# zhaoweicai/mscnn

Measured on AMD Instinct MI355X. Metric: images/sec mscnn-7s-576 KITTI-car inference, higher is better.
Workload: dtype f32

## Files before the change

### include/mscnn_hip.h

```cpp
#ifndef MSCNN_HIP_H_
#define MSCNN_HIP_H_

#include <stddef.h>
#include <stdint.h>

#if defined(__GNUC__)
#define MSCNN_API __attribute__((visibility("default")))
#else
#define MSCNN_API
#endif

#ifdef __cplusplus
extern "C" {
#endif

typedef enum {
  MSCNN_OK = 0,
  MSCNN_ERR_BAD_ARG = 1,
  MSCNN_ERR_HIP = 2,
  MSCNN_ERR_WORKSPACE = 3,
  MSCNN_ERR_UNSUPPORTED = 4
} mscnn_status;

MSCNN_API const char* mscnn_last_error(void);
// ... 31 lines not shown
MSCNN_API int mscnn_conv2d_plan_plane_columns(const mscnn_conv_plan* plan, int* cols, int n);
MSCNN_API int mscnn_conv2d_plan_set_profiling(mscnn_conv_plan* plan, int on);
MSCNN_API int mscnn_conv2d_plan_stage_ms(const mscnn_conv_plan* plan, float ms_out[3]);
#define MSCNN_AMAX_SLOTS 1024
MSCNN_API int mscnn_conv2d_plan_publishes_amax(const mscnn_conv_plan* plan);
MSCNN_API int mscnn_conv2d_plan_set_amax_io(mscnn_conv_plan* plan, const uint32_t* in_bound, uint32_t* out_amax);
MSCNN_API int mscnn_conv2d_plan_set_batch(mscnn_conv_plan* plan, int N);
MSCNN_API unsigned long long mscnn_conv2d_plan_weight_layout(const mscnn_conv_plan* plan);
MSCNN_API int mscnn_conv2d_pack_weights(const mscnn_conv_plan* plan, const float* w, float* packed, void* stream);
MSCNN_API int mscnn_conv2d_fwd_f32(const mscnn_conv_plan* plan, const float* x, const float* w, const float* packed,
                         const float* bias, float* y, void* workspace, size_t workspace_bytes, void* stream);
MSCNN_API int mscnn_conv2d_plan_can_pool(const mscnn_conv_plan* plan);
MSCNN_API int mscnn_conv2d_fwd_pool_f32(const mscnn_conv_plan* plan, const float* x, const float* w, const float* packed,
                              const float* bias, float* y, float* y_pool, void* workspace, size_t workspace_bytes,
                              void* stream);

MSCNN_API int mscnn_relu_fwd_f32(const float* x, float* y, size_t count, float negative_slope, void* stream);

MSCNN_API int mscnn_pool_out_dim(int in, int kernel, int pad, int stride);
MSCNN_API int mscnn_pool2d_fwd_f32(const float* x, float* y, int N, int C, int H, int W, int kernel_h, int kernel_w,
                         int pad_h, int pad_w, int stride_h, int stride_w, int method, void* stream);

MSCNN_API int mscnn_inner_product_fwd_f32(const float* x, const float* w, const float* bias, float* y,
                                int M, int N, int K, int relu, void* stream);
MSCNN_API void mscnn_debug_inner_product_rows(int rows);

MSCNN_API int mscnn_inner_product_wg_supported(int M, int N, int K);
MSCNN_API size_t mscnn_inner_product_wg_packed_bytes(int N, int K);
MSCNN_API size_t mscnn_inner_product_wg_workspace_bytes(int M, int N, int K);
MSCNN_API int mscnn_inner_product_wg_pack(const float* w, float* wt, int N, int K, void* stream);
MSCNN_API int mscnn_inner_product_wg_fwd(const float* x, const float* wt, const float* bias, float* y, int M, int N, int K, int relu,
                                         void* workspace, size_t workspace_bytes, void* stream);
MSCNN_API unsigned long long mscnn_wgemm_handoff_event(void);
MSCNN_API void mscnn_wgemm_force_whole_tiles(int on);
MSCNN_API int mscnn_wgemm_whole_tiles_forced(void);
MSCNN_API void mscnn_debug_wgemm_handoff_fault(int drop_publish, unsigned spin_limit);
MSCNN_API long mscnn_debug_wgemm_schedule(const mscnn_conv_plan* plan, int whole_tiles, int* rows, long max_rows, int info[8]);
MSCNN_API int mscnn_inner_product_x3_supported(int N, int K);
MSCNN_API size_t mscnn_inner_product_x3_packed_bytes(int N, int K);
MSCNN_API size_t mscnn_inner_product_x3_workspace_bytes(int M, int N, int K);
MSCNN_API int mscnn_inner_product_x3_pack(const float* w, void* packed, int N, int K, void* stream);
MSCNN_API int mscnn_inner_product_x3_fwd(const float* x, const void* packed, const float* bias, float* y, int M, int N, int K, int relu,
                               const uint32_t* in_bound, void* workspace, size_t workspace_bytes, void* stream);
MSCNN_API int mscnn_inner_product_f16_supported(int N, int K);
MSCNN_API int mscnn_inner_product_pack_f16(const float* w, void* w16, int N, int K, void* stream);
MSCNN_API int mscnn_inner_product_fwd_f16(const float* x, const void* w16, const float* bias, float* y, int M, int N, int K, int relu,
                                          void* stream);

MSCNN_API int mscnn_concat_channels_f32(const float* x, float* y, int N, int C, int inner, int C_total, int c_offset, void* stream);

MSCNN_API int mscnn_deconv_depthwise_fwd_f32(const float* x, const float* w, const float* bias, float* y,
                                   int N, int C, int H, int W, int Kh, int Kw, int pad_h, int pad_w,
                                   int stride_h, int stride_w, void* stream);

MSCNN_API int mscnn_deconv2d_fwd_f32(const float* x, const float* w, const float* bias, float* y, int N, int Cin, int H, int W,
                                     int Cout, int Kh, int Kw, int pad_h, int pad_w, int stride_h, int stride_w, int group,
                                     void* stream);

MSCNN_API int mscnn_max_rel_diff_f32(const float* a, const float* ref, size_t count, float floor, float* out_dev, void* stream);
MSCNN_API int mscnn_max_rel_diff_strided_f32(const float* a, size_t a_stride, const float* ref, size_t ref_stride, size_t planes, size_t run,
                                             const double* sumsq_dev, double sumsq_count, float* out_dev, void* stream);
MSCNN_API int mscnn_store_words_i32(int* dst_dev, const int* values_host, int n, void* stream);
MSCNN_API int mscnn_sum_squares_f32(const float* x, size_t count, double* out_dev, void* stream);

MSCNN_API int mscnn_softmax_fwd_f32(const float* x, float* y, int outer, int C, int inner, void* stream);

MSCNN_API int mscnn_roipool_fwd_f32(const float* feat, const float* rois, float* out, int R, int N, int C, int H, int W,
                          int pooled_h, int pooled_w, float spatial_scale, float pad_ratio,
                          int C_total, int c_offset, void* stream);
MSCNN_API int mscnn_roipool_pair_fwd_f32(const float* feat, const float* rois, float* out, int R, int N, int C, int H, int W,
                                         int pooled_h, int pooled_w, float spatial_scale, float pad_ratio_a, int c_offset_a,
                                         float pad_ratio_b, int c_offset_b, int C_total, void* stream);

MSCNN_API int mscnn_conv2d_plan_can_chain(const mscnn_conv_plan* plan, const mscnn_conv_plan* next);
MSCNN_API int mscnn_conv2d_plan_can_pool_only(const mscnn_conv_plan* plan);
MSCNN_API int mscnn_conv2d_fwd_chain_f32(const mscnn_conv_plan* plan, const mscnn_conv_plan* next, const float* x, const float* packed,
                               const float* bias, float* y, float* y_pool, void* workspace, size_t workspace_bytes,
                               void* next_workspace, size_t next_workspace_bytes, void* stream);

MSCNN_API int mscnn_conv2d_plan_can_fuse_roipool(const mscnn_conv_plan* plan, int C, int pooled_h, int pooled_w);
MSCNN_API size_t mscnn_conv2d_roipool_workspace_bytes(const mscnn_conv_plan* plan, int N, int C, int H, int W);
MSCNN_API size_t mscnn_roipool_maps_bytes(int N, int C, int H, int W);
MSCNN_API int mscnn_roipool_maps_build_f32(const float* feat, float* maps, int N, int C, int H, int W, void* stream);
MSCNN_API int mscnn_conv2d_fwd_roipool_pair_f32(const mscnn_conv_plan* plan, const float* feat, const float* prepared_maps, int N, int C,
                                                int H, int W, const float* rois, float spatial_scale, float pad_ratio_a,
                                                float pad_ratio_b, const float* packed_w, const float* bias, float* y, void* workspace,
                                                size_t workspace_bytes, void* stream);

MSCNN_API int mscnn_roialign_fwd_f32(const float* feat, const float* rois, float* out, int R, int N, int C, int H, int W,
                                     int pooled_h, int pooled_w, float spatial_scale, float pad_ratio, void* stream);
MSCNN_API int mscnn_roialign_ave_fwd_f32(const float* feat, const float* rois, float* out, int R, int N, int C, int H, int W,
                                         int pooled_h, int pooled_w, float spatial_scale, float pad_ratio,
                                         int C_total, int c_offset, void* stream);
MSCNN_API int mscnn_roialign_ave_pair_fwd_f32(const float* feat, const float* rois, float* out, int R, int N, int C, int H, int W,
                                              int pooled_h, int pooled_w, float spatial_scale, float pad_ratio_a, int c_offset_a,
                                              float pad_ratio_b, int c_offset_b, int C_total, void* stream);

MSCNN_API int mscnn_eltwise_fwd_f32(const float* const* bottoms_host, int num_bottoms, const float* coeffs_host, float* y,
                                    size_t count, int op, void* stream);

#define MSCNN_BOXOUT_MAX_HEADS 16
typedef struct {
  int num_heads;
  int num;
  int channels;
  int head_h[MSCNN_BOXOUT_MAX_HEADS], head_w[MSCNN_BOXOUT_MAX_HEADS];
  float field_w[MSCNN_BOXOUT_MAX_HEADS], field_h[MSCNN_BOXOUT_MAX_HEADS], downsample_rate[MSCNN_BOXOUT_MAX_HEADS];
  float fg_thr, iou_thr;
  int nms_mode;
  float field_whr, field_xyr;
  int max_nms_num, max_post_nms_num;
  float min_size;
  int do_bbox_norm;
  float bbox_mean[4], bbox_std[4];
} mscnn_boxoutput_desc;

MSCNN_API size_t mscnn_boxoutput_workspace_bytes(const mscnn_boxoutput_desc* desc);
MSCNN_API int mscnn_boxoutput_max_rows(const mscnn_boxoutput_desc* desc);
MSCNN_API int mscnn_boxoutput_fwd_f32(const mscnn_boxoutput_desc* desc, const float* const* heads_host,
                            float* rois_out, float* props_out, int* anchor_ids_out, int cap,
                            int* count_out_dev, void* workspace, size_t workspace_bytes, void* stream);
MSCNN_API size_t mscnn_boxoutput_batch_workspace_bytes(const mscnn_boxoutput_desc* desc);
MSCNN_API int mscnn_boxoutput_batch_fwd_f32(const mscnn_boxoutput_desc* desc, const float* const* heads_host,
                            float* rois_out, float* props_out, int* anchor_ids_out, int cap,
                            int* count_out_dev, void* workspace, size_t workspace_bytes, void* stream);

MSCNN_API size_t mscnn_nms_workspace_bytes(int n);
MSCNN_API int mscnn_nms_greedy_f32(const float* boxes_xywh, int n, float iou_thr, int nms_mode, unsigned char* keep_out,
                         void* workspace, size_t workspace_bytes, void* stream);

MSCNN_API int mscnn_decodebbox_fwd_f32(const float* bbox, const float* prior, float* out, int R, int bbox_dim,
                             const float* mean_host, const float* std_host, void* stream);

typedef struct {
  int ncls, cls_id;
  float bbox_mean[4], bbox_std[4];
  float proposal_thr;
  double ratio_h, ratio_w, org_h, org_w, nms_overlap;
} mscnn_detections_desc;
MSCNN_API size_t mscnn_detections_workspace_bytes(int R);

enum { MSCNN_NMS_TYPE_MAXG = 0, MSCNN_NMS_TYPE_MAX = 1, MSCNN_NMS_TYPE_MS = 2, MSCNN_NMS_TYPE_COVER = 3, MSCNN_NMS_TYPE_NONE = 4 };
enum { MSCNN_NMS_OVR_UNION = 0, MSCNN_NMS_OVR_MIN = 1 };
#ifndef MSCNN_NMS_PARAMS_DEFINED
#define MSCNN_NMS_PARAMS_DEFINED
typedef struct {
  int type;
  int ovr_dnm;
  double thr;
  float det_thr;
} mscnn_nms_params;
#endif
MSCNN_API int mscnn_nms_params_resolve(const mscnn_nms_params* nms, mscnn_nms_params* out);
MSCNN_API int mscnn_nms_params_from_names(const char* type, const char* ovr_dnm, double thr, double maxn, float det_thr,
                                          mscnn_nms_params* out);
MSCNN_API int mscnn_detections_fwd(const mscnn_detections_desc* desc, const float* bbox_pred, const float* cls_pred,
                         const float* props, int R, double* dets_out, int* ids_out, int* count_out_dev,
                         void* workspace, size_t workspace_bytes, void* stream);

MSCNN_API int mscnn_detections_nms_fwd(const mscnn_detections_desc* desc, const mscnn_nms_params* nms, const float* bbox_pred,
                                       const float* cls_pred, const float* props, int R, double* dets_out, int* ids_out,
                                       int* count_out_dev, void* workspace, size_t workspace_bytes, void* stream);

MSCNN_API int mscnn_detections_cascade_fwd(const mscnn_detections_desc* desc, float det_thr, const float* boxes,
                                 const float* cls_prob, const float* props, int R, double* dets_out, int* ids_out,
                                 int* count_out_dev, void* workspace, size_t workspace_bytes, void* stream);
// ... 123 lines not shown
```

### mscnn_amd/csrc/roipool_wino.hip

```cpp
#include "roipool_wino.h"
#include "wino33_device.h"
#include <cfloat>

namespace {

typedef unsigned u32x4 __attribute__((ext_vector_type(4)));
typedef unsigned u32x2 __attribute__((ext_vector_type(2)));

constexpr int kNB = 4;
constexpr int kLevels = 4;

struct RpwArgs {
  const float* maps;
  const float* rois;
  float* V;
  int R, C, H, W, T_pad;
  unsigned level_bytes, maps_bytes, v_bytes;
  float spatial_scale, pad_a, pad_b;
};

__device__ __forceinline__ __amdgpu_buffer_rsrc_t make_rsrc(const void* p, unsigned bytes) {
  return __builtin_amdgcn_make_buffer_rsrc(const_cast<void*>(p), 0, (int)bytes, 0x00020000);
}
__device__ __forceinline__ int uni(int v) { return __builtin_amdgcn_readfirstlane(v); }
// ... 157 lines not shown
      }
      __syncthreads();
#pragma unroll
      for (int j = 0; j < 5; ++j) {
        float* slot_ = &s_out[(j * 64 + lane) * kLdsRow + wave * 4];
        if (!RAG || (i < 4 && j < 4)) *reinterpret_cast<float4*>(slot_) = make_float4(out[j][0], out[j][1], out[j][2], out[j][3]);
        else if (i < 4) *reinterpret_cast<float2*>(slot_) = make_float2(out[j][0], out[j][2]);
        else if (j < 4) *reinterpret_cast<float2*>(slot_) = make_float2(out[j][0], out[j][1]);
        else *slot_ = out[j][0];
      }
      __syncthreads();
      static_assert(kRois == 8, "thread = (channel, roi) of a pass");
#pragma unroll
      for (int j = 0; j < 5; ++j) {
        const int rq = tid % kRois, ch = tid / kRois;
        if (r0 + rq < a.R) {
          const float* unit = &s_out[(j * 64 + ch) * kLdsRow + rq * 4];
          const int uw = RAG ? (i < 4 ? 2 : 1) * (j < 4 ? 2 : 1) : 4;
          const unsigned off = (unsigned)(i * 5 + j) * plane_bytes + ((unsigned)(q * C + c0 + ch) * (unsigned)a.T_pad + (unsigned)(r0 + rq) * (unsigned)uw) * 4u;
#ifdef RPW_NO_STORE
          if (a.T_pad < 0)
#endif
          {
            if (uw == 4) {
              const float4 u = *reinterpret_cast<const float4*>(unit);
              u32x4 pk;
              pk.x = __builtin_bit_cast(unsigned, u.x); pk.y = __builtin_bit_cast(unsigned, u.y);
              pk.z = __builtin_bit_cast(unsigned, u.z); pk.w = __builtin_bit_cast(unsigned, u.w);
              __builtin_amdgcn_raw_buffer_store_b128(pk, rV, off, 0u, 0);
            } else if (uw == 2) {
              const float2 u = *reinterpret_cast<const float2*>(unit);
              u32x2 pk;
              pk.x = __builtin_bit_cast(unsigned, u.x); pk.y = __builtin_bit_cast(unsigned, u.y);
              __builtin_amdgcn_raw_buffer_store_b64(pk, rV, off, 0u, 0);
            } else {
              __builtin_amdgcn_raw_buffer_store_b32(__builtin_bit_cast(unsigned, unit[0]), rV, off, 0u, 0);
            }
          }
        }
      }
    }
  }
}

__global__ __launch_bounds__(256) void nchw_to_nhwc_kernel(const float* __restrict__ x, float* __restrict__ y, int C, int HW) {
  __shared__ float t[64][65];
  const int n = blockIdx.z, c0 = blockIdx.y * 64, p0 = blockIdx.x * 64;
  const int tx = threadIdx.x & 63, ty = threadIdx.x >> 6;
  const float* src = x + (size_t)n * C * HW;
  float* dst = y + (size_t)n * C * HW;
#pragma unroll
  for (int i = 0; i < 16; ++i) {
    const int cc = c0 + ty + 4 * i, pp = p0 + tx;
    t[ty + 4 * i][tx] = (cc < C && pp < HW) ? src[(size_t)cc * HW + pp] : 0.f;
  }
  __syncthreads();
#pragma unroll
  for (int i = 0; i < 16; ++i) {
    const int pp = p0 + ty + 4 * i, cc = c0 + tx;
    if (pp < HW && cc < C) dst[(size_t)pp * C + cc] = t[tx][ty + 4 * i];
  }
}

__global__ __launch_bounds__(256) void sliding_max_kernel(const float* __restrict__ src, float* __restrict__ dst, int H, int W, int C4, int half,
                                                          long total) {
  const long i = blockIdx.x * 256L + threadIdx.x;
  if (i >= total) return;
  const int c4 = (int)(i % C4);
  long p = i / C4;
  const int x = (int)(p % W); p /= W;
  const int y = (int)(p % H);
  const long n = p / H;
  const int y2 = min(y + half, H - 1), x2 = min(x + half, W - 1);
  const float4* s4 = reinterpret_cast<const float4*>(src) + n * H * W * C4;
  const float4 a = s4[((long)y * W + x) * C4 + c4], b = s4[((long)y * W + x2) * C4 + c4];
  const float4 c = s4[((long)y2 * W + x) * C4 + c4], d = s4[((long)y2 * W + x2) * C4 + c4];
  float4 m = a;
  m.x = b.x > m.x ? b.x : m.x; m.y = b.y > m.y ? b.y : m.y; m.z = b.z > m.z ? b.z : m.z; m.w = b.w > m.w ? b.w : m.w;
  m.x = c.x > m.x ? c.x : m.x; m.y = c.y > m.y ? c.y : m.y; m.z = c.z > m.z ? c.z : m.z; m.w = c.w > m.w ? c.w : m.w;
  m.x = d.x > m.x ? d.x : m.x; m.y = d.y > m.y ? d.y : m.y; m.z = d.z > m.z ? d.z : m.z; m.w = d.w > m.w ? d.w : m.w;
  reinterpret_cast<float4*>(dst)[i] = m;
}

}

namespace mscnn {

bool roipool_wino33_supported(int C, int pooled_h, int pooled_w, int conv_pad_h, int conv_pad_w) {
  return pooled_h == 7 && pooled_w == 7 && conv_pad_h == 0 && conv_pad_w == 0 && C > 0 && C % 64 == 0;
}

size_t roipool_wino33_scratch_bytes(int N, int C, int H, int W) { return (size_t)kLevels * N * C * H * W * sizeof(float); }

int roipool_wino33_build_maps(const float* feat, float* maps, int N, int C, int H, int W, hipStream_t st) {
  MSCNN_REQUIRE(feat && maps, "roipool maps: null pointer");
  MSCNN_REQUIRE(N > 0 && C % 64 == 0 && H > 0 && W > 0, "roipool maps: bad shape");
  MSCNN_REQUIRE(kLevels * (double)N * C * H * W * 4.0 < 4.0e9, "roipool maps: beyond a 32-bit buffer window");
  MSCNN_REQUIRE(reinterpret_cast<uintptr_t>(maps) % 16 == 0, "roipool maps: the maps must be 16-byte aligned");
  const int HW = H * W;
  const long per_level = (long)N * C * HW;
  nchw_to_nhwc_kernel<<<dim3(cdiv(HW, 64), cdiv(C, 64), N), 256, 0, st>>>(feat, maps, C, HW);
  MSCNN_POST_LAUNCH();
  for (int k = 1; k < kLevels; ++k) {
    const long total = per_level / 4;
    sliding_max_kernel<<<(unsigned)((total + 255) / 256), 256, 0, st>>>(maps + (k - 1) * per_level, maps + k * per_level, H, W, C / 4, 1 << (k - 1), total);
    MSCNN_POST_LAUNCH();
  }
  return MSCNN_OK;
}

int roipool_wino33_forward(const float* maps, const float* rois, float* V, int R, int N, int C, int H, int W, int T_pad,
                           float spatial_scale, float pad_a, float pad_b, hipStream_t st, int ragged) {
  MSCNN_REQUIRE(maps && rois && V, "roipool+transform: null pointer");
  MSCNN_REQUIRE(ragged == 0 || ragged == wino33_ragged_mode(5, 5), "roipool+transform: the planes are uniform or ragged on both axes (5 x 5 outputs)");
  MSCNN_REQUIRE(R > 0 && N > 0 && C % 64 == 0 && H > 0 && W > 0 && T_pad >= 4 * R && T_pad % 4 == 0, "roipool+transform: bad shape");
  const double lb = (double)N * C * H * W * 4.0, vb = 25.0 * 2.0 * C * (double)T_pad * 4.0;
  MSCNN_REQUIRE(kLevels * lb < 4.0e9 && vb < 4.0e9, "roipool+transform: feature maps or transform planes beyond a 32-bit buffer window");
  MSCNN_REQUIRE(reinterpret_cast<uintptr_t>(V) % 16 == 0, "roipool+transform: V must be 16-byte aligned");
  RpwArgs a;
  a.maps = maps; a.rois = rois; a.V = V;
  a.R = R; a.C = C; a.H = H; a.W = W; a.T_pad = T_pad;
  a.level_bytes = (unsigned)lb; a.maps_bytes = (unsigned)(kLevels * lb); a.v_bytes = (unsigned)vb;
  a.spatial_scale = spatial_scale; a.pad_a = pad_a; a.pad_b = pad_b;
  if (ragged) roipool_wino33_kernel<7, 7, true><<<dim3(C / 64, cdiv(R, kRois), 2), kRois * 64, 0, st>>>(a);
  else roipool_wino33_kernel<7, 7, false><<<dim3(C / 64, cdiv(R, kRois), 2), kRois * 64, 0, st>>>(a);
  MSCNN_POST_LAUNCH();
  return MSCNN_OK;
}

}
```

### mscnn_amd/hipapi.py

```python
import ctypes as C
import os

import numpy as np
import torch

_HERE = os.path.dirname(os.path.abspath(__file__))
LIB_PATH = os.path.join(_HERE, "libmscnn_hip.so")
_lib = None


class MscnnError(RuntimeError):
    pass


class ConvDesc(C.Structure):
    _fields_ = [(n, C.c_int) for n in ("N", "Cin", "H", "W", "Cout", "Kh", "Kw", "pad_h", "pad_w",
                                       "stride_h", "stride_w", "group", "relu", "algo", "tune_variant", "tune_grid", "tune_flags")]


AMAX_SLOTS = 1024
ALGO_AUTO, ALGO_DIRECT, ALGO_WINO_F2, ALGO_WINO_F3, ALGO_F16, ALGO_WINO_F3_X3, ALGO_WINO_F4 = 0, 1, 2, 3, 4, 5, 6


MAX_HEADS = 16
# ... 41 lines not shown
NMS_NULL = object()


def _nms_ref(nms):
    if nms is NMS_NULL:
        return None
    return C.byref(nms if isinstance(nms, NmsParams) else nms_params(**nms))


def lib():
    global _lib
    if _lib is None:
        if not os.path.exists(LIB_PATH):
            raise MscnnError(f"{LIB_PATH} not built: run `python -c 'import __graft_entry__ as g; g.build()'`")
        L = C.CDLL(LIB_PATH)
        L.mscnn_last_error.restype = C.c_char_p
        L.mscnn_version.restype = C.c_char_p
        L.mscnn_conv2d_plan_kernel.restype = C.c_char_p
        L.mscnn_conv2d_plan_kernel.argtypes = [C.c_void_p]
        L.mscnn_conv2d_plan_publishes_amax.argtypes = [C.c_void_p]
        L.mscnn_conv2d_plan_set_amax_io.argtypes = [C.c_void_p, C.c_void_p, C.c_void_p]
        L.mscnn_conv2d_plan_dtype.restype = C.c_char_p
        L.mscnn_conv2d_plan_dtype.argtypes = [C.c_void_p]
        L.mscnn_inner_product_f16_supported.argtypes = [C.c_int, C.c_int]
        L.mscnn_inner_product_x3_supported.argtypes = [C.c_int, C.c_int]
        L.mscnn_inner_product_x3_packed_bytes.restype = C.c_size_t
        L.mscnn_inner_product_x3_packed_bytes.argtypes = [C.c_int, C.c_int]
        L.mscnn_inner_product_x3_workspace_bytes.restype = C.c_size_t
        L.mscnn_inner_product_x3_workspace_bytes.argtypes = [C.c_int] * 3
        L.mscnn_inner_product_x3_pack.argtypes = [C.c_void_p, C.c_void_p, C.c_int, C.c_int, C.c_void_p]
        L.mscnn_inner_product_x3_fwd.argtypes = [C.c_void_p] * 4 + [C.c_int] * 4 + [C.c_void_p, C.c_void_p, C.c_size_t, C.c_void_p]
        L.mscnn_inner_product_wg_supported.argtypes = [C.c_int] * 3
        L.mscnn_inner_product_wg_packed_bytes.restype = C.c_size_t
        L.mscnn_inner_product_wg_packed_bytes.argtypes = [C.c_int, C.c_int]
        L.mscnn_inner_product_wg_workspace_bytes.restype = C.c_size_t
        L.mscnn_inner_product_wg_workspace_bytes.argtypes = [C.c_int] * 3
        L.mscnn_inner_product_wg_pack.argtypes = [C.c_void_p, C.c_void_p, C.c_int, C.c_int, C.c_void_p]
        L.mscnn_inner_product_wg_fwd.argtypes = [C.c_void_p] * 4 + [C.c_int] * 4 + [C.c_void_p, C.c_size_t, C.c_void_p]
        L.mscnn_max_rel_diff_f32.argtypes = [C.c_void_p, C.c_void_p, C.c_size_t, C.c_float, C.c_void_p, C.c_void_p]
        L.mscnn_sum_squares_f32.argtypes = [C.c_void_p, C.c_size_t, C.c_void_p, C.c_void_p]
        L.mscnn_max_rel_diff_strided_f32.argtypes = [C.c_void_p, C.c_size_t, C.c_void_p, C.c_size_t, C.c_size_t, C.c_size_t, C.c_void_p, C.c_double,
                                                     C.c_void_p, C.c_void_p]
        L.mscnn_store_words_i32.argtypes = [C.c_void_p, C.c_void_p, C.c_int, C.c_void_p]
        L.mscnn_wgemm_handoff_event.restype = C.c_ulonglong
        L.mscnn_wgemm_handoff_event.argtypes = []
        L.mscnn_wgemm_force_whole_tiles.restype = None
        L.mscnn_wgemm_force_whole_tiles.argtypes = [C.c_int]
        L.mscnn_wgemm_whole_tiles_forced.argtypes = []
        L.mscnn_debug_inner_product_rows.restype = None
        L.mscnn_debug_inner_product_rows.argtypes = [C.c_int]
        L.mscnn_debug_wgemm_handoff_fault.restype = None
        L.mscnn_debug_wgemm_handoff_fault.argtypes = [C.c_int, C.c_uint]
        L.mscnn_inner_product_pack_f16.argtypes = [C.c_void_p, C.c_void_p, C.c_int, C.c_int, C.c_void_p]
        L.mscnn_inner_product_fwd_f16.argtypes = [C.c_void_p] * 4 + [C.c_int] * 4 + [C.c_void_p]
        for f in ("mscnn_conv2d_plan_flops", "mscnn_conv2d_plan_executed_flops"):
            getattr(L, f).restype = C.c_double
            getattr(L, f).argtypes = [C.c_void_p]
        L.mscnn_conv2d_plan_set_profiling.argtypes = [C.c_void_p, C.c_int]
        L.mscnn_conv2d_plan_plane_columns.argtypes = [C.c_void_p, C.c_void_p, C.c_int]
        L.mscnn_debug_wgemm_schedule.restype = C.c_long
        L.mscnn_debug_wgemm_schedule.argtypes = [C.c_void_p, C.c_int, C.c_void_p, C.c_long, C.c_void_p]
        L.mscnn_conv2d_plan_stage_ms.argtypes = [C.c_void_p, C.c_void_p]
        for f in ("mscnn_conv2d_packed_weight_bytes", "mscnn_conv2d_workspace_bytes"):
            getattr(L, f).restype = C.c_size_t
            getattr(L, f).argtypes = [C.c_void_p]
        L.mscnn_conv2d_plan_destroy.argtypes = [C.c_void_p]
        L.mscnn_conv2d_plan_destroy.restype = None
        L.mscnn_conv2d_plan_set_batch.argtypes = [C.c_void_p, C.c_int]
        L.mscnn_conv2d_pack_weights.argtypes = [C.c_void_p] * 4
        L.mscnn_conv2d_fwd_f32.argtypes = [C.c_void_p] * 7 + [C.c_size_t, C.c_void_p]
        L.mscnn_conv2d_fwd_pool_f32.argtypes = [C.c_void_p] * 8 + [C.c_size_t, C.c_void_p]
        L.mscnn_conv2d_plan_can_pool.argtypes = [C.c_void_p]
        L.mscnn_conv2d_plan_can_fuse_roipool.argtypes = [C.c_void_p, C.c_int, C.c_int, C.c_int]
        L.mscnn_conv2d_plan_can_chain.argtypes = [C.c_void_p, C.c_void_p]
        L.mscnn_conv2d_plan_can_pool_only.argtypes = [C.c_void_p]
        L.mscnn_conv2d_fwd_chain_f32.argtypes = [C.c_void_p] * 8 + [C.c_size_t, C.c_void_p, C.c_size_t, C.c_void_p]
        L.mscnn_conv2d_roipool_workspace_bytes.restype = C.c_size_t
        L.mscnn_conv2d_roipool_workspace_bytes.argtypes = [C.c_void_p] + [C.c_int] * 4
        L.mscnn_conv2d_fwd_roipool_pair_f32.argtypes = ([C.c_void_p, C.c_void_p, C.c_void_p] + [C.c_int] * 4 + [C.c_void_p, C.c_float, C.c_float, C.c_float]
                                                        + [C.c_void_p] * 4 + [C.c_size_t, C.c_void_p])
        L.mscnn_roipool_maps_bytes.restype = C.c_size_t
        L.mscnn_roipool_maps_bytes.argtypes = [C.c_int] * 4
        L.mscnn_roipool_maps_build_f32.argtypes = [C.c_void_p, C.c_void_p] + [C.c_int] * 4 + [C.c_void_p]
        L.mscnn_conv2d_plan_weight_layout.argtypes = [C.c_void_p]
        L.mscnn_conv2d_plan_weight_layout.restype = C.c_ulonglong
        L.mscnn_relu_fwd_f32.argtypes = [C.c_void_p, C.c_void_p, C.c_size_t, C.c_float, C.c_void_p]
        L.mscnn_pool2d_fwd_f32.argtypes = [C.c_void_p, C.c_void_p] + [C.c_int] * 11 + [C.c_void_p]
        L.mscnn_inner_product_fwd_f32.argtypes = [C.c_void_p] * 4 + [C.c_int] * 4 + [C.c_void_p]
        L.mscnn_concat_channels_f32.argtypes = [C.c_void_p, C.c_void_p] + [C.c_int] * 5 + [C.c_void_p]
        L.mscnn_deconv_depthwise_fwd_f32.argtypes = [C.c_void_p] * 4 + [C.c_int] * 10 + [C.c_void_p]
        L.mscnn_softmax_fwd_f32.argtypes = [C.c_void_p, C.c_void_p, C.c_int, C.c_int, C.c_int, C.c_void_p]
        L.mscnn_roipool_fwd_f32.argtypes = ([C.c_void_p] * 3 + [C.c_int] * 7 + [C.c_float, C.c_float] + [C.c_int] * 2
                                            + [C.c_void_p])
        L.mscnn_roipool_pair_fwd_f32.argtypes = ([C.c_void_p] * 3 + [C.c_int] * 7 + [C.c_float, C.c_float, C.c_int, C.c_float, C.c_int, C.c_int]
                                                 + [C.c_void_p])
        L.mscnn_roialign_fwd_f32.argtypes = [C.c_void_p] * 3 + [C.c_int] * 7 + [C.c_float, C.c_float, C.c_void_p]
        L.mscnn_roialign_ave_fwd_f32.argtypes = ([C.c_void_p] * 3 + [C.c_int] * 7 + [C.c_float, C.c_float] + [C.c_int] * 2
                                                 + [C.c_void_p])
        L.mscnn_roialign_ave_pair_fwd_f32.argtypes = ([C.c_void_p] * 3 + [C.c_int] * 7
                                                      + [C.c_float, C.c_float, C.c_int, C.c_float, C.c_int, C.c_int] + [C.c_void_p])
        L.mscnn_eltwise_fwd_f32.argtypes = [C.c_void_p, C.c_int, C.c_void_p, C.c_void_p, C.c_size_t, C.c_int, C.c_void_p]
        L.mscnn_boxoutput_workspace_bytes.restype = C.c_size_t
        L.mscnn_boxoutput_workspace_bytes.argtypes = [C.c_void_p]
        L.mscnn_boxoutput_max_rows.argtypes = [C.c_void_p]
        L.mscnn_boxoutput_fwd_f32.argtypes = [C.c_void_p, C.c_void_p, C.c_void_p, C.c_void_p, C.c_void_p, C.c_int,
                                              C.c_void_p, C.c_void_p, C.c_size_t, C.c_void_p]
        L.mscnn_boxoutput_batch_workspace_bytes.restype = C.c_size_t
        L.mscnn_boxoutput_batch_workspace_bytes.argtypes = [C.c_void_p]
        L.mscnn_boxoutput_batch_fwd_f32.argtypes = L.mscnn_boxoutput_fwd_f32.argtypes
        L.mscnn_nms_workspace_bytes.restype = C.c_size_t
        L.mscnn_nms_workspace_bytes.argtypes = [C.c_int]
        L.mscnn_nms_greedy_f32.argtypes = [C.c_void_p, C.c_int, C.c_float, C.c_int, C.c_void_p, C.c_void_p, C.c_size_t,
                                           C.c_void_p]
        L.mscnn_decodebbox_fwd_f32.argtypes = [C.c_void_p] * 3 + [C.c_int, C.c_int, C.c_void_p, C.c_void_p, C.c_void_p]
        L.mscnn_detections_workspace_bytes.restype = C.c_size_t
        L.mscnn_detections_workspace_bytes.argtypes = [C.c_int]
        L.mscnn_detections_fwd.argtypes = [C.c_void_p] * 4 + [C.c_int] + [C.c_void_p] * 4 + [C.c_size_t, C.c_void_p]
        L.mscnn_detections_multi_pack_bytes.restype = C.c_size_t
        L.mscnn_detections_multi_pack_bytes.argtypes = [C.c_int, C.c_int]
        L.mscnn_detections_multi_workspace_bytes.restype = C.c_size_t
        L.mscnn_detections_multi_workspace_bytes.argtypes = [C.c_int, C.c_int]
        L.mscnn_detections_multi_fwd.argtypes = ([C.c_void_p, C.c_int, C.c_int] + [C.c_void_p] * 3 + [C.c_int, C.c_int, C.c_void_p, C.c_int,
                                                 C.c_void_p, C.c_size_t, C.c_void_p])
        L.mscnn_detections_cascade_multi_workspace_bytes.restype = C.c_size_t
        L.mscnn_detections_cascade_multi_workspace_bytes.argtypes = [C.c_int, C.c_int]
        L.mscnn_detections_cascade_multi_fwd.argtypes = ([C.c_void_p, C.c_float, C.c_int, C.c_int, C.c_int, C.c_void_p, C.c_int, C.c_int,
                                                         C.c_void_p, C.c_int, C.c_void_p, C.c_size_t, C.c_void_p])
        L.mscnn_nms_params_resolve.argtypes = [C.c_void_p, C.c_void_p]
        L.mscnn_nms_params_from_names.argtypes = [C.c_char_p, C.c_char_p, C.c_double, C.c_double, C.c_float, C.c_void_p]
        L.mscnn_detections_nms_fwd.argtypes = [C.c_void_p] * 5 + [C.c_int] + [C.c_void_p] * 4 + [C.c_size_t, C.c_void_p]
        L.mscnn_detections_cascade_nms_fwd.argtypes = ([C.c_void_p, C.c_float] + [C.c_void_p] * 4 + [C.c_int] + [C.c_void_p] * 4 +
                                                       [C.c_size_t, C.c_void_p])
        L.mscnn_detections_multi_nms_fwd.argtypes = ([C.c_void_p, C.c_void_p, C.c_int, C.c_int] + [C.c_void_p] * 3 +
                                                     [C.c_int, C.c_int, C.c_void_p, C.c_int, C.c_void_p, C.c_size_t, C.c_void_p])
        L.mscnn_detections_cascade_multi_nms_fwd.argtypes = ([C.c_void_p, C.c_float, C.c_void_p, C.c_int, C.c_int, C.c_int, C.c_void_p,
                                                              C.c_int, C.c_int, C.c_void_p, C.c_int, C.c_void_p, C.c_size_t, C.c_void_p])
        L.mscnn_detections_candidates_bytes.restype = C.c_size_t
        L.mscnn_detections_candidates_bytes.argtypes = [C.c_int, C.c_int]
        L.mscnn_detections_candidates_reset.argtypes = [C.c_void_p, C.c_int, C.c_int, C.c_void_p]
        L.mscnn_detections_candidates_add.argtypes = ([C.c_void_p] * 3 + [C.c_int] * 3 + [C.c_void_p] * 3 +
                                                      [C.c_int, C.c_void_p, C.c_int, C.c_void_p])
        L.mscnn_detections_candidates_cascade_add.argtypes = ([C.c_void_p, C.c_void_p, C.c_float, C.c_void_p] + [C.c_int] * 4 +
                                                              [C.c_void_p, C.c_int, C.c_void_p, C.c_int, C.c_void_p])
        L.mscnn_detections_candidates_add_views.argtypes = ([C.c_void_p] * 4 + [C.c_int] * 4 + [C.c_void_p] * 3 +
                                                            [C.c_int, C.c_void_p, C.c_int, C.c_void_p])
        L.mscnn_detections_candidates_cascade_add_views.argtypes = ([C.c_void_p, C.c_void_p, C.c_void_p, C.c_float, C.c_void_p] + [C.c_int] * 5 +
                                                                    [C.c_void_p, C.c_int, C.c_void_p, C.c_int, C.c_void_p])
        L.mscnn_preprocess_views_workspace_bytes.restype = C.c_size_t
        L.mscnn_preprocess_views_workspace_bytes.argtypes = [C.c_void_p, C.c_int, C.c_int, C.c_int]
        L.mscnn_preprocess_views_u8_f32.argtypes = ([C.c_void_p, C.c_void_p, C.c_void_p, C.c_int, C.c_void_p, C.c_int, C.c_void_p, C.c_int, C.c_int,
                                                     C.c_void_p, C.c_void_p, C.c_size_t, C.c_void_p])
        L.mscnn_detections_merge_workspace_bytes.restype = C.c_size_t
        L.mscnn_detections_merge_workspace_bytes.argtypes = [C.c_int, C.c_int]
        L.mscnn_detections_merge_fwd.argtypes = [C.c_void_p, C.c_void_p, C.c_int, C.c_void_p, C.c_int, C.c_void_p, C.c_void_p, C.c_size_t,
                                                 C.c_void_p]
        L.mscnn_detections_merge_vote_fwd.argtypes = [C.c_void_p, C.c_int, C.c_void_p, C.c_int, C.c_void_p, C.c_void_p]
        L.mscnn_detections_merge_soft_workspace_bytes.restype = C.c_size_t
        L.mscnn_detections_merge_soft_workspace_bytes.argtypes = [C.c_int, C.c_int]
        L.mscnn_detections_merge_soft_fwd.argtypes = [C.c_void_p, C.c_void_p, C.c_int, C.c_void_p, C.c_int, C.c_void_p, C.c_void_p, C.c_size_t,
                                                      C.c_void_p]
        L.mscnn_detections_merge_matrix_workspace_bytes.restype = C.c_size_t
        L.mscnn_detections_merge_matrix_workspace_bytes.argtypes = [C.c_int, C.c_int]
        L.mscnn_detections_merge_matrix_fwd.argtypes = [C.c_void_p, C.c_int, C.c_void_p, C.c_int, C.c_void_p, C.c_void_p, C.c_size_t, C.c_void_p]
        L.mscnn_proposals_multi_pack_bytes.restype = C.c_size_t
        L.mscnn_proposals_multi_pack_bytes.argtypes = [C.c_int, C.c_int]
        L.mscnn_proposals_multi_fwd.argtypes = [C.c_void_p, C.c_int, C.c_void_p, C.c_int, C.c_void_p, C.c_int, C.c_void_p]
# ... 833 lines not shown
        S, cap = self.S, self.cap
        ov = self.overlap if nms_overlap is None else nms_overlap
        ov = (C.c_double * S)(*[float(v) for v in (ov if ov is not None else [0.5] * S)])
        nbytes = lib().mscnn_detections_multi_pack_bytes(S, S * cap)
        if pack is None:
            pack = torch.zeros(nbytes, dtype=torch.uint8, device=self.buf.device)
        wb = lib().mscnn_detections_merge_workspace_bytes(S, cap)
        if ws is None:
            ws = torch.empty(max(wb, 1), dtype=torch.uint8, device=self.buf.device)
        _check(lib().mscnn_detections_merge_fwd(ov, _nms_ref(nms), S, _dev(self.buf), cap, _dev(pack), _dev(ws), C.c_size_t(ws.numel()),
                                                _stream()))
        if vote_thr is not None:
            self.vote(pack, vote_thr)
        return self._read_pack(pack, nbytes, raw_pack, "detections_merge")

    def merge_soft(self, method, sigma=0.5, score_thr=0.001, max_out=0, nms_overlap=None, raw_pack=False, pack=None, ws=None, vote_thr=None):
        S, cap = self.S, self.cap
        ov = self.overlap if nms_overlap is None else nms_overlap
        ov = (C.c_double * S)(*[float(v) for v in (ov if ov is not None else [0.5] * S)])
        nbytes = lib().mscnn_detections_multi_pack_bytes(S, S * cap)
        if pack is None:
            pack = torch.zeros(nbytes, dtype=torch.uint8, device=self.buf.device)
        wb = lib().mscnn_detections_merge_soft_workspace_bytes(S, cap)
        if ws is None:
            ws = torch.empty(max(wb, 1), dtype=torch.uint8, device=self.buf.device)
        soft = SoftNmsParams(soft_nms_method(method), float(sigma), float(score_thr), int(max_out))
        _check(lib().mscnn_detections_merge_soft_fwd(ov, C.byref(soft), S, _dev(self.buf), cap, _dev(pack), _dev(ws), C.c_size_t(ws.numel()),
                                                     _stream()))
        if vote_thr is not None:
            self.vote(pack, vote_thr)
        return self._read_pack(pack, nbytes, raw_pack, "detections_merge_soft")

    def merge_matrix(self, method, sigma=0.5, score_thr=0.001, max_out=0, raw_pack=False, pack=None, ws=None, vote_thr=None):
        S, cap = self.S, self.cap
        nbytes = lib().mscnn_detections_multi_pack_bytes(S, S * cap)
        if pack is None:
            pack = torch.zeros(nbytes, dtype=torch.uint8, device=self.buf.device)
        wb = lib().mscnn_detections_merge_matrix_workspace_bytes(S, cap)
        if ws is None:
            ws = torch.empty(max(wb, 1), dtype=torch.uint8, device=self.buf.device)
        mx = MatrixNmsParams(matrix_nms_method(method), float(sigma), float(score_thr), int(max_out))
        _check(lib().mscnn_detections_merge_matrix_fwd(C.byref(mx), S, _dev(self.buf), cap, _dev(pack), _dev(ws), C.c_size_t(ws.numel()),
                                                       _stream()))
        if vote_thr is not None:
            self.vote(pack, vote_thr)
        return self._read_pack(pack, nbytes, raw_pack, "detections_merge_matrix")

    def _read_pack(self, pack, nbytes, raw_pack, what):
        S, cap = self.S, self.cap
        h = pack[:nbytes].cpu().numpy()
        table = 16 * (S + 1)
        hdr = h[:table].view(np.int32).reshape(S + 1, 4)
        if list(hdr[0]) != [S, cap, S * cap, 0]:
            raise MscnnError(f"{what}: pack header {hdr[0].tolist()}")
        dets = h[table:table + 40 * S * cap].view(np.float64).reshape(-1, 5)
        tags = h[table + 40 * S * cap:table + 44 * S * cap].view(np.int32)
        out = []
        for s in range(S):
            cnt, cands, row0, zero = (int(v) for v in hdr[1 + s])
            if row0 != s * cap or zero != 0:
                raise MscnnError(f"{what}: table entry {s}: {hdr[1 + s].tolist()}")
            out.append((dets[row0:row0 + cnt].copy(), tags[row0:row0 + cnt].copy(), cands) if cnt >= 0 else (None, None, cands))
        return (out, h) if raw_pack else out


def wgemm_handoff_event():
    return int(lib().mscnn_wgemm_handoff_event())


def wgemm_force_whole_tiles(on=True):
    lib().mscnn_wgemm_force_whole_tiles(int(bool(on)))


def wgemm_whole_tiles_forced():
    return bool(lib().mscnn_wgemm_whole_tiles_forced())


def debug_wgemm_handoff_fault(drop_publish=False, spin_limit=0):
    lib().mscnn_debug_wgemm_handoff_fault(int(bool(drop_publish)), int(spin_limit))


def debug_inner_product_rows(rows=0):
    lib().mscnn_debug_inner_product_rows(int(rows))
```

Baseline: 230.2.

## Build ROI-pool max-pyramid maps in one fused LDS-tiled kernel

Replaces the four-launch pyramid build (NCHW-to-NHWC transpose plus three sliding-max passes, each reading the prior level from global memory) with a single kernel. Each block loads a channel-block spatial tile with a halo into LDS and computes all four levels in place. It writes every level straight to global memory in NHWC. This removes three launches and the global re-reads of intermediate levels, at the cost of halo overlap, large LDS use that may lower occupancy, and strided channel writes. The old path stays reachable through a debug switch.

Measured after the change: 231.3 (median of 6 runs). No clear change (+0.5%).

```diff
diff --git a/include/mscnn_hip.h b/include/mscnn_hip.h
--- a/include/mscnn_hip.h
+++ b/include/mscnn_hip.h
@@ -137,6 +137,7 @@
 MSCNN_API size_t mscnn_conv2d_roipool_workspace_bytes(const mscnn_conv_plan* plan, int N, int C, int H, int W);
 MSCNN_API size_t mscnn_roipool_maps_bytes(int N, int C, int H, int W);
 MSCNN_API int mscnn_roipool_maps_build_f32(const float* feat, float* maps, int N, int C, int H, int W, void* stream);
+MSCNN_API void mscnn_debug_roipool_maps_form(int form);
 MSCNN_API int mscnn_conv2d_fwd_roipool_pair_f32(const mscnn_conv_plan* plan, const float* feat, const float* prepared_maps, int N, int C,
                                                 int H, int W, const float* rois, float spatial_scale, float pad_ratio_a,
                                                 float pad_ratio_b, const float* packed_w, const float* bias, float* y, void* workspace,
diff --git a/mscnn_amd/csrc/roipool_wino.hip b/mscnn_amd/csrc/roipool_wino.hip
--- a/mscnn_amd/csrc/roipool_wino.hip
+++ b/mscnn_amd/csrc/roipool_wino.hip
@@ -263,7 +263,121 @@
   reinterpret_cast<float4*>(dst)[i] = m;
 }
 
-}
+constexpr int seg_of(int rows) {
+  for (int s = 8; s > 1; --s)
+    if (rows % s == 0) return s;
+  return 1;
+}
+
+template <int CB, int TH, int TW, int NT>
+struct MapsTile {
+  static constexpr int RH = TH + 7, RW = TW + 7, LS = CB + 1, SLOTS = NT / CB;
+  static constexpr int lds_floats = RH * RW * LS;
+  static_assert(NT % CB == 0 && CB % 32 == 0 && lds_floats * 4 <= 160 * 1024, "tile");
+};
+
+struct MapsArgs {
+  const float* feat;
+  float* maps;
+  int C, H, W, tiles_x;
+  size_t per_level;
+};
+
+template <int CB, int TH, int TW, int NT, int HALF>
+__device__ __forceinline__ void maps_level(float* s, const MapsArgs& a, float* g0, int c, int slot, int y0, int x0) {
+  using T = MapsTile<CB, TH, TW, NT>;
+  constexpr int RHO = TH + 8 - 2 * HALF, RWO = TW + 8 - 2 * HALF, SEG = seg_of(RHO), ITEMS = RWO * (RHO / SEG);
+  constexpr int ITER = (ITEMS + T::SLOTS - 1) / T::SLOTS, K = HALF == 1 ? 1 : HALF == 2 ? 2 : 3;
+  float out[ITER][SEG];
+#pragma unroll
+  for (int it = 0; it < ITER; ++it) {
+    const int item = slot + it * T::SLOTS;
+    if (item < ITEMS) {
+      const int seg = item / RWO, lx = item - seg * RWO, ly0 = seg * SEG;
+      const float* col = s + (ly0 * T::RW + lx) * T::LS + c;
+      float va[SEG + HALF], vb[SEG + HALF];
+#pragma unroll
+      for (int r = 0; r < SEG + HALF; ++r) {
+        va[r] = col[r * T::RW * T::LS];
+        vb[r] = col[(r * T::RW + HALF) * T::LS];
+      }
+      const bool col_live = lx < TW && x0 + lx < a.W;
+      float* g = g0 + ((size_t)(y0 + ly0) * a.W + (x0 + lx)) * a.C;
+#pragma unroll
+      for (int r = 0; r < SEG; ++r) {
+        float m = va[r];
+        m = vb[r] > m ? vb[r] : m;
+        m = va[r + HALF] > m ? va[r + HALF] : m;
+        m = vb[r + HALF] > m ? vb[r + HALF] : m;
+        out[it][r] = m;
+        if (col_live && ly0 + r < TH && y0 + ly0 + r < a.H) {
+          float* px = g + (size_t)r * a.W * a.C;
+          if (HALF == 1) px[0] = va[r];
+          px[(size_t)K * a.per_level] = m;
+        }
+      }
+    }
+  }
+  if (HALF < 4) {
+    __syncthreads();
+#pragma unroll
+    for (int it = 0; it < ITER; ++it) {
+      const int item = slot + it * T::SLOTS;
+      if (item < ITEMS) {
+        const int seg = item / RWO, lx = item - seg * RWO, ly0 = seg * SEG;
+        float* col = s + (ly0 * T::RW + lx) * T::LS + c;
+#pragma unroll
+        for (int r = 0; r < SEG; ++r) col[r * T::RW * T::LS] = out[it][r];
+      }
+    }
+    __syncthreads();
+  }
+}
+
+template <int CB, int TH, int TW, int NT>
+__global__ __launch_bounds__(NT) void roipool_maps_one_pass_kernel(MapsArgs a) {
+  using T = MapsTile<CB, TH, TW, NT>;
+  __shared__ float s_maps[T::lds_floats];
+  const int tid = threadIdx.x;
+  const int c0 = blockIdx.x * CB, n = blockIdx.z;
+  const int ty = blockIdx.y / a.tiles_x, tx = blockIdx.y - ty * a.tiles_x;
+  const int y0 = ty * TH, x0 = tx * TW;
+  const int H = a.H, W = a.W;
+  const float* src = a.feat + ((size_t)n * a.C + c0) * H * W;
+  constexpr int kCells = T::RH * T::RW, kTotal = CB * kCells;
+#pragma unroll 4
+  for (int i = tid; i < kTotal; i += NT) {
+    const int cc = i / kCells, p = i - cc * kCells;
+    const int ly = p / T::RW, lx = p - ly * T::RW;
+    const int gy = min(y0 + ly, H - 1), gx = min(x0 + lx, W - 1);
+    s_maps[p * T::LS + cc] = src[((size_t)cc * H + gy) * W + gx];
+  }
+  __syncthreads();
+  const int c = tid % CB, slot = tid / CB;
+  float* g0 = a.maps + (size_t)n * H * W * a.C + c0 + c;
+  maps_level<CB, TH, TW, NT, 1>(s_maps, a, g0, c, slot, y0, x0);
+  maps_level<CB, TH, TW, NT, 2>(s_maps, a, g0, c, slot, y0, x0);
+  maps_level<CB, TH, TW, NT, 4>(s_maps, a, g0, c, slot, y0, x0);
+}
+
+template <int CB, int TH, int TW, int NT>
+int launch_maps_one_pass(const float* feat, float* maps, int N, int C, int H, int W, hipStream_t st) {
+  MapsArgs a;
+  a.feat = feat; a.maps = maps; a.C = C; a.H = H; a.W = W;
+  a.tiles_x = mscnn::cdiv(W, TW);
+  a.per_level = (size_t)N * C * H * W;
+  const int tiles = a.tiles_x * mscnn::cdiv(H, TH);
+  MSCNN_REQUIRE(tiles <= 65535 && N <= 65535, "roipool maps: more tiles or images than a grid axis holds");
+  roipool_maps_one_pass_kernel<CB, TH, TW, NT><<<dim3(C / CB, tiles, N), NT, 0, st>>>(a);
+  MSCNN_POST_LAUNCH();
+  return MSCNN_OK;
+}
+
+int g_maps_form = 0;
+
+}
+
+extern "C" void mscnn_debug_roipool_maps_form(int form) { g_maps_form = form == 1 ? 1 : 0; }
 
 namespace mscnn {
 
@@ -278,6 +392,7 @@
   MSCNN_REQUIRE(N > 0 && C % 64 == 0 && H > 0 && W > 0, "roipool maps: bad shape");
   MSCNN_REQUIRE(kLevels * (double)N * C * H * W * 4.0 < 4.0e9, "roipool maps: beyond a 32-bit buffer window");
   MSCNN_REQUIRE(reinterpret_cast<uintptr_t>(maps) % 16 == 0, "roipool maps: the maps must be 16-byte aligned");
+  if (g_maps_form == 0) return launch_maps_one_pass<32, 12, 24, 512>(feat, maps, N, C, H, W, st);
   const int HW = H * W;
   const long per_level = (long)N * C * HW;
   nchw_to_nhwc_kernel<<<dim3(cdiv(HW, 64), cdiv(C, 64), N), 256, 0, st>>>(feat, maps, C, HW);
diff --git a/mscnn_amd/hipapi.py b/mscnn_amd/hipapi.py
--- a/mscnn_amd/hipapi.py
+++ b/mscnn_amd/hipapi.py
@@ -147,6 +147,8 @@
         L.mscnn_roipool_maps_bytes.restype = C.c_size_t
         L.mscnn_roipool_maps_bytes.argtypes = [C.c_int] * 4
         L.mscnn_roipool_maps_build_f32.argtypes = [C.c_void_p, C.c_void_p] + [C.c_int] * 4 + [C.c_void_p]
+        L.mscnn_debug_roipool_maps_form.restype = None
+        L.mscnn_debug_roipool_maps_form.argtypes = [C.c_int]
         L.mscnn_conv2d_plan_weight_layout.argtypes = [C.c_void_p]
         L.mscnn_conv2d_plan_weight_layout.restype = C.c_ulonglong
         L.mscnn_relu_fwd_f32.argtypes = [C.c_void_p, C.c_void_p, C.c_size_t, C.c_float, C.c_void_p]
@@ -1146,3 +1148,7 @@
 
 def debug_inner_product_rows(rows=0):
     lib().mscnn_debug_inner_product_rows(int(rows))
+
+
+def debug_roipool_maps_form(form=0):
+    lib().mscnn_debug_roipool_maps_form(int(form))
```
